# ai-forever/Kandinsky-2

Measured on NVIDIA H100. Metric: unet_denoising_steps_per_sec, higher is better.
Workload: dtype f16

## Files before the change

kandinsky-2_b200/csrc/k2_api.cu:

```cuda
#include <stdio.h>
#include <stdlib.h>
#include <string.h>

#include <algorithm>
#include <atomic>
#include <mutex>

#include "../../include/k2b200.h"
#include "k2_internal.h"

namespace k2 {

static thread_local std::string g_err;
static std::atomic<long long> g_launches{0};
static int g_force_bn = 0;
static int g_force_split = 0;
static int g_pdl = 0;


void set_error(const std::string& msg) { g_err = msg; }
int fail(const std::string& msg) {
  g_err = msg;
  return -1;
}
// ... 77 lines not shown
      for (int k = (tn == 1 ? 0 : 1); k < 2; ++k) {
        bool better = best_tiles[k] < 0 || tiles < best_tiles[k];
        if (!better && tiles == best_tiles[k]) {
          if (tn != bn[k]) {
            better = tn < bn[k];
          } else {
            const int d_new = tw > th ? tw - th : th - tw;
            const int d_old = bw[k] > bh[k] ? bw[k] - bh[k] : bh[k] - bw[k];
            better = (d_new < d_old) || (d_new == d_old && tw > bw[k]);
          }
        }
        if (better) {
          best_tiles[k] = tiles;
          bn[k] = tn;
          bw[k] = tw;
          bh[k] = th;
        }
      }
    }
  }
  const int k = (!single_image_only && best_tiles[1] * 100 <= best_tiles[0] * 85) ? 1 : 0;
  TN = bn[k];
  TW = bw[k];
  TH = bh[k];
}


struct ConvPlan {
  int TN, TH, TW, tiles_w, tiles_h, tiles_n, m_tiles;
  int m_tiles_phase;
  int BN, splits;
  int fuse_stats, row_groups;
  int es;
};

static void plan_conv(int NB, int H, int W, bool any9, int kchunks, int Cout, int out_mode, bool has_workspace,
                      long long workspace_bytes, bool want_gn, ConvPlan& pl, const int* cfg = nullptr, bool up2 = false,
                      bool w_batched = false) {
  const int g_force_bn = (cfg && cfg[0]) ? cfg[0] : k2::g_force_bn;
  const int g_force_split = (cfg && cfg[2]) ? cfg[2] : k2::g_force_split;
  pl.es = (cfg && cfg[3]) ? cfg[3] : k2::g_conv_epi_sets;
  choose_tile(NB, H, W, pl.TN, pl.TH, pl.TW, w_batched);
  pl.tiles_w = (W + pl.TW - 1) / pl.TW;
  pl.tiles_h = (H + pl.TH - 1) / pl.TH;
  pl.tiles_n = (NB + pl.TN - 1) / pl.TN;
  pl.m_tiles = pl.tiles_w * pl.tiles_h * pl.tiles_n;
  pl.m_tiles_phase = pl.m_tiles;

  int BN = g_force_bn;
  int splits = 1;
  const long long M_total = static_cast<long long>(NB) * H * W;
  const bool can_split = !up2 && !w_batched && has_workspace && out_mode == 0 && Cout % 8 == 0;
  auto split_ok = [&](int sp) {
    if (sp == 1) return true;
    const int kps = (kchunks + sp - 1) / sp;
    return can_split && kps >= 8 && (sp - 1) * kps < kchunks &&
           static_cast<long long>(sp) * M_total * Cout * 4 <= workspace_bytes;
  };
  auto model = [&](int bn, int sp) {
    const long long nt = (Cout + bn - 1) / bn;
    const long long units = static_cast<long long>(pl.m_tiles) * nt * sp * (up2 ? 4 : 1);
    const long long slots = num_sms();
    const long long waves = (units + slots - 1) / slots;
    const long long kps = (kchunks + sp - 1) / sp;
    long long cost = waves * (kps * (4LL * bn + 60) + 2000);
    if (sp > 1) cost += 4000 + (static_cast<long long>(sp) + 1) * M_total * Cout * 4 / 1800;
    return cost;
  };
  if (BN == 0) {
    if (Cout <= 16) BN = 16;
    else if (Cout <= 64) BN = 64;
    else if (Cout <= 128) BN = 128;
    else BN = 0;
  }
  {
    const int cand[3] = {256, 192, 128};
    long long best = -1;
    int best_bn = BN ? BN : 256, best_sp = 1;
    for (int ci = 0; ci < 3; ++ci) {
      const int bn = BN ? BN : cand[ci];
      if (BN && ci > 0) break;
      for (int sp = 1; sp <= 8; ++sp) {
        if (g_force_split > 0 && sp != g_force_split) continue;
        if (!split_ok(sp)) continue;
        const long long c = model(bn, sp);
        if (best < 0 || c < best) {
          best = c;
          best_bn = bn;
          best_sp = sp;
        }
      }
    }
    BN = best_bn;
    splits = best_sp;
  }
  pl.BN = BN;
  pl.splits = splits;

  pl.fuse_stats = 0;
  pl.row_groups = 0;
  if (want_gn && out_mode == 0 && Cout % 8 == 0) {
    if (splits == 1 && BN >= 64 && Cout % 64 == 0 && (pl.TN == 1 || pl.TH * pl.TW == 16)) {
      pl.fuse_stats = 1;
      pl.row_groups = ((pl.TN == 1) ? pl.m_tiles : NB * pl.tiles_h * pl.tiles_w) * (up2 ? 4 : 1);
    } else if (splits > 1 && (static_cast<long long>(H) * W) % 16 == 0) {
      pl.fuse_stats = 2;
      pl.row_groups = static_cast<int>(M_total / 16);
    }
  }
}

static void plan_to_info(const ConvPlan& pl, int* info) {
  if (!info) return;
  info[0] = pl.BN; info[1] = 0;
  info[2] = pl.splits; info[3] = pl.m_tiles; info[4] = pl.TN;
  info[5] = pl.fuse_stats; info[6] = pl.row_groups;
}

}

using namespace k2;

extern "C" {

const char* k2_last_error(void) { return g_err.c_str(); }
int k2_version(void) { return 100; }
long long k2_launch_count(void) { return g_launches.load(); }
void k2_reset_launch_count(void) { g_launches.store(0); }
int k2_set_tuning(int key, int value) {
  if (key == 0) {
    g_force_bn = value;
    return 0;
  }
  if (key == 1) {
    g_force_split = value;
    return 0;
  }
  if (key == 2) {
    if (value == 2) return fail("k2_set_tuning: no CTA-pair conv kernel on sm_90");
    return 0;
  }
  if (key == 4) {
    g_pdl = value;
    return 0;
  }
  if (key == 10) {
    g_conv_epi_sets = (value == 2) ? 2 : 1;
    return 0;
  }
  if (key == 11) {
    g_gn_bps = value;
    return 0;
  }
  if (key == 9) {
    return 0;
  }

  return fail("k2_set_tuning: unknown key");
}

int k2_conv_gemm(const K2ConvSrc* srcs, int nsrc, int NB, int H, int W, const void* w_packed, int w_rows,
                 int Ktot, int ldw, int Cout, const float* bias, const void* residual, int ldr, void* out, int ldo,
                 int out_mode, void* workspace, long long workspace_bytes, float* gn_partial, int* info,
                 k2_stream_t stream) {
  return k2_conv_gemm_cfg(srcs, nsrc, NB, H, W, w_packed, w_rows, Ktot, ldw, Cout, bias, residual, ldr, out, ldo, out_mode,
                          workspace, workspace_bytes, gn_partial, info, nullptr, 0, stream);
}

int k2_conv_gemm_cfg(const K2ConvSrc* srcs, int nsrc, int NB, int H, int W, const void* w_packed, int w_rows,
                     int Ktot, int ldw, int Cout, const float* bias, const void* residual, int ldr, void* out, int ldo,
                     int out_mode, void* workspace, long long workspace_bytes, float* gn_partial, int* info,
                     const int* cfg, long long w_batch_stride, k2_stream_t stream) {
  K2_REQUIRE(w_batch_stride >= 0 && w_batch_stride % 8 == 0, "conv_gemm_cfg: w_batch_stride must be a multiple of 8 elements");
  const bool w_batched = w_batch_stride > 0;
  if (cfg) {
    K2_REQUIRE(cfg[0] == 0 || cfg[0] == 16 || cfg[0] == 64 || cfg[0] == 128 || cfg[0] == 192 || cfg[0] == 256,
               "conv_gemm_cfg: N tile must be 0, 16, 64, 128, 192 or 256");
    K2_REQUIRE(cfg[1] >= 0 && cfg[1] <= 2 && cfg[2] >= 0 && cfg[2] <= 8 && cfg[3] >= 0 && cfg[3] <= 2,
               "conv_gemm_cfg: pair mode in 0..2, splits in 0..8, epilogue sets in 0..2");
    K2_REQUIRE(cfg[1] != 2, "conv_gemm_cfg: no CTA-pair conv kernel on sm_90");
  }
  K2_REQUIRE(nsrc >= 1 && nsrc <= 3, "conv_gemm: 1..3 sources");
  K2_REQUIRE((reinterpret_cast<uintptr_t>(gn_partial) & 7) == 0, "conv_gemm: gn_partial must be 8-byte aligned");
  K2_REQUIRE(NB > 0 && H > 0 && W > 0 && Cout > 0, "conv_gemm: bad geometry");
  K2_REQUIRE(w_rows >= Cout, "conv_gemm: w_rows < Cout");
  K2_REQUIRE(Ktot % 64 == 0, "conv_gemm: Ktot must be a multiple of 64");
  if (ldw == 0) ldw = Ktot;
  K2_REQUIRE(ldw >= Ktot && ldw % 8 == 0 && (reinterpret_cast<uintptr_t>(w_packed) & 15) == 0,
             "conv_gemm: weight row stride / alignment");
  ConvGemmParams p;
  memset(&p, 0, sizeof p);
  p.NB = NB;
  p.H = H;
  p.W = W;
  bool any9 = false;
  int kchunks = 0;
  const bool up2 = srcs[0].taps == 4;
  if (up2) {
    K2_REQUIRE(nsrc == 1 && out_mode == 0 && residual == nullptr && H % 2 == 0 && W % 2 == 0,
               "conv_gemm: a taps == 4 source (3x3 conv over its nearest-2x upsampling) must be the only source, with fp16 "
               "output, no residual and even output H, W");
    H /= 2;
    W /= 2;
    p.H = H;
    p.W = W;
  }
  for (int s = 0; s < nsrc; ++s) {
    const K2ConvSrc& src = srcs[s];
    K2_REQUIRE(src.taps == 9 || src.taps == 1 || (s == 0 && src.taps == 4), "conv_gemm: taps must be 9 or 1 (or 4: up2)");
    K2_REQUIRE(src.C > 0 && src.C % 8 == 0 && src.ld % 8 == 0 && src.ld >= src.C, "conv_gemm: bad source C/ld");
    K2_REQUIRE((reinterpret_cast<uintptr_t>(src.ptr) & 15) == 0, "conv_gemm: source not 16B aligned");
    any9 = any9 || src.taps == 9;
    p.seg_taps[s] = src.taps;
// ... 26 lines not shown
                        static_cast<uint64_t>(NB)};
    uint64_t str[3] = {static_cast<uint64_t>(src.ld) * 2, static_cast<uint64_t>(src.ld) * 2 * W,
                       static_cast<uint64_t>(src.ld) * 2 * W * H};
    uint32_t box[4] = {64, static_cast<uint32_t>(p.TW), static_cast<uint32_t>(p.TH), static_cast<uint32_t>(p.TN)};
    if (encode_tmap_f16(&p.tmA[s], src.ptr, 4, dims, str, box)) return -1;
  }
  const int BN = pl.BN, splits = pl.splits, fuse_stats = pl.fuse_stats;
  p.splits = splits;
  p.k_per_split = (kchunks + splits - 1) / splits;
  p.M_total = static_cast<long long>(NB) * H * W * (up2 ? 4 : 1);
  p.ws = reinterpret_cast<float*>(workspace);
  p.n_tiles = (Cout + BN - 1) / BN;
  p.Cout = Cout;
  {
    uint64_t dims[3] = {static_cast<uint64_t>(Ktot), static_cast<uint64_t>(w_rows), static_cast<uint64_t>(w_batched ? NB : 1)};
    uint64_t str[2] = {static_cast<uint64_t>(ldw) * 2,
                       (w_batched ? static_cast<uint64_t>(w_batch_stride) : static_cast<uint64_t>(ldw) * w_rows) * 2};
    uint32_t box[3] = {64, static_cast<uint32_t>(BN), 1};
    if (encode_tmap_f16(&p.tmB, w_packed, 3, dims, str, box)) return -1;
  }
  p.bias = bias;
  p.residual = reinterpret_cast<const __half*>(residual);
  p.ldr = ldr;
  p.out = out;
  p.ldo = ldo;
  p.out_mode = (splits > 1) ? 2 : out_mode;
  p.gn_part = (fuse_stats == 1) ? reinterpret_cast<float2*>(gn_partial) : nullptr;
  p.gn_mode = (fuse_stats == 1) ? (p.TN == 1 ? 1 : 2) : 0;
  if (out_mode == 0) {
    K2_REQUIRE(ldo % 8 == 0 && (reinterpret_cast<uintptr_t>(out) & 15) == 0, "conv_gemm: out alignment");
    if (residual)
      K2_REQUIRE(ldr % 8 == 0 && (reinterpret_cast<uintptr_t>(residual) & 15) == 0, "conv_gemm: residual alignment");
  }
  int rc = launch_conv_gemm(p, BN, pl.es, static_cast<cudaStream_t>(stream));
  if (rc == 0) g_launches.fetch_add(1, std::memory_order_relaxed);
  if (rc == 0 && splits > 1) {
    rc = launch_splitk_finalize(p.ws, splits, p.M_total, Cout, bias, p.residual, ldr, reinterpret_cast<__half*>(out), ldo,
                                fuse_stats == 2 ? reinterpret_cast<float2*>(gn_partial) : nullptr,
                                static_cast<cudaStream_t>(stream));
    if (rc == 0) g_launches.fetch_add(1, std::memory_order_relaxed);
  }
  return rc;
}

int k2_conv_plan(int NB, int H, int W, int taps, int Ktot, int Cout, int out_mode, long long workspace_bytes,
                 int want_gn_partial, int* info) {
  K2_REQUIRE(NB > 0 && H > 0 && W > 0 && Cout > 0 && info, "conv_plan: bad arguments");
  K2_REQUIRE(Ktot > 0 && Ktot % 64 == 0, "conv_plan: Ktot must be a positive multiple of 64");
  ConvPlan pl;
  plan_conv(NB, H, W, taps == 9, Ktot / 64, Cout, out_mode, workspace_bytes > 0, workspace_bytes, want_gn_partial != 0, pl);
  plan_to_info(pl, info);
  return 0;
}

}
```

kandinsky-2_b200/csrc/k2_conv_gemm.cu:

```cuda
#include <stdio.h>

#include "k2_common.cuh"
#include "k2_internal.h"

namespace k2 {

namespace {

constexpr int BM = 128;
constexpr int BK = 64;
constexpr int A_STAGE_BYTES = BM * BK * 2;
constexpr int ACC_PAD = 4;

constexpr int EPI_STAGE_FLOATS = 32 * 33;
constexpr int EPI_BYTES = 4 * EPI_STAGE_FLOATS * 4 + 4 * 256 * 4;
constexpr int SMEM_LIMIT = 227 * 1024;

template <int BN, int ES>
struct Cfg {
  static constexpr int B_STAGE_BYTES = BN * BK * 2;
  static constexpr int STAGE_BYTES = A_STAGE_BYTES + B_STAGE_BYTES;
  static constexpr int BNC = (BN < 64) ? BN : (ES == 2 ? 128 : 64);
  static_assert(ES == 1 || BN % 128 == 0, "two epilogue sets need N tiles of 128 or 256");
  static constexpr int ACC_BYTES = BM * (BNC + ACC_PAD) * 4;
// ... 280 lines not shown
                uint4 ov;
                __half2* oh = reinterpret_cast<__half2*>(&ov);
#pragma unroll
                for (int e = 0; e < 4; ++e) oh[e] = __floats2half2_rn(f[2 * e], f[2 * e + 1]);
                *reinterpret_cast<uint4*>(orow + v * 8) = ov;
              }
            } else {
#pragma unroll
              for (int e = 0; e < CH; ++e) {
                if (col0 + e < p.Cout) {
                  float f = __uint_as_float(r[e]);
                  if (p.bias) f += __ldg(p.bias + col0 + e);
                  if (rrow) f += __half2float(rrow[e]);
                  orow[e] = __float2half_rn(f);
                }
              }
            }
          } else {
            float* o = reinterpret_cast<float*>(p.out);
#pragma unroll
            for (int e = 0; e < CH; ++e) {
              if (col0 + e < p.Cout) {
                float f = __uint_as_float(r[e]);
                if (p.bias) f += __ldg(p.bias + col0 + e);
                o[((static_cast<long long>(n) * p.Cout + (col0 + e)) * p.H + y) * p.W + x] = f;
              }
            }
          }
        }
      }
}


template <int BN, int ES>
__global__ void __launch_bounds__(384, 1) conv_gemm_kernel(const __grid_constant__ ConvGemmParams p) {
  using C = Cfg<BN, ES>;
  constexpr int BNC = C::BNC;
  constexpr int NA = BN / 2;
  extern __shared__ uint8_t smem_raw[];
  uint8_t* smem = reinterpret_cast<uint8_t*>((reinterpret_cast<uintptr_t>(smem_raw) + 1023) &
                                             ~static_cast<uintptr_t>(1023));
  float* acc_smem = reinterpret_cast<float*>(smem + C::STAGES * C::STAGE_BYTES);
  float* stat_smem = reinterpret_cast<float*>(smem + C::STAGES * C::STAGE_BYTES + C::ACC_BYTES);
  uint64_t* full_bar = reinterpret_cast<uint64_t*>(smem + C::STAGES * C::STAGE_BYTES + C::ACC_BYTES + ES * EPI_BYTES);
  uint64_t* empty_bar = full_bar + C::STAGES;

  const int warp_idx = threadIdx.x >> 5;
  const int lane = threadIdx.x & 31;
  const int wg = warp_idx >> 2;

  if (threadIdx.x == 0) {
    tma_prefetch_desc(&p.tmB);
    for (int s = 0; s < 3; ++s)
      if (p.seg_taps[s]) tma_prefetch_desc(&p.tmA[s]);
    for (int i = 0; i < C::STAGES; ++i) {
      mbar_init(&full_bar[i], 1);
      mbar_init(&empty_bar[i], 8);
    }
    fence_barrier_init();
  }
  __syncthreads();
  pdl_wait();
  pdl_launch();

  const int total_tiles = p.m_tiles * p.n_tiles * p.splits;

  if (wg == 0) {
    setmaxnreg_dec<40>();
    if (warp_idx == 0 && elect_one()) {
      int stage = 0;
      uint32_t ring_phase = 0;
      const uint32_t tx_bytes = p.a_box_bytes + C::B_STAGE_BYTES;
      for (int tile = blockIdx.x; tile < total_tiles; tile += gridDim.x) {
        const int m_idx = tile % p.m_tiles;
        const int n_idx = (tile / p.m_tiles) % p.n_tiles;
        const int split = tile / (p.m_tiles * p.n_tiles);
        int n0, y0, x0, phase;
        decode_m_tile(p, m_idx, n0, y0, x0, phase);
        const int kb = phase * p.num_k_chunks;
        const int k0 = split * p.k_per_split;
        const int k1 = min(p.num_k_chunks, k0 + p.k_per_split);
        int s = 0, rem = k0;
        while (rem >= p.seg_taps[s] * p.seg_kchunks[s]) {
          rem -= p.seg_taps[s] * p.seg_kchunks[s];
          ++s;
        }
        int tap = rem / p.seg_kchunks[s];
        int c = rem - tap * p.seg_kchunks[s];
        for (int kc = k0; kc < k1; ++kc) {
          const int taps = p.seg_taps[s];
          const int dy = (taps == 9) ? (tap / 3 - 1) : (taps == 4 ? (tap >> 1) + (phase >> 1) - 1 : 0);
          const int dx = (taps == 9) ? (tap % 3 - 1) : (taps == 4 ? (tap & 1) + (phase & 1) - 1 : 0);
          mbar_wait_lean(&empty_bar[stage], ring_phase ^ 1);
          uint8_t* sA = smem + stage * C::STAGE_BYTES;
          uint8_t* sB = sA + A_STAGE_BYTES;
          mbar_arrive_expect_tx(&full_bar[stage], tx_bytes);
          tma_load_4d(sA, &p.tmA[s], &full_bar[stage], c * BK, x0 + dx, y0 + dy, n0);
          tma_load_3d(sB, &p.tmB, &full_bar[stage], (kb + kc) * BK, n_idx * BN, p.w_batched ? n0 : 0);
          if (++stage == C::STAGES) {
            stage = 0;
            ring_phase ^= 1;
          }
          if (++c == p.seg_kchunks[s]) {
            c = 0;
            if (++tap == taps) {
              tap = 0;
              ++s;
            }
          }
        }
      }
    }
  } else {
    setmaxnreg_inc<232>();
    const int g = wg - 1;
    const int w = warp_idx & 3;
    int stage = 0;
    uint32_t phase = 0;
    for (int tile = blockIdx.x; tile < total_tiles; tile += gridDim.x) {
      const int m_idx = tile % p.m_tiles;
      const int n_idx = (tile / p.m_tiles) % p.n_tiles;
      const int split = tile / (p.m_tiles * p.n_tiles);
      const int nk = min(p.num_k_chunks, (split + 1) * p.k_per_split) - split * p.k_per_split;
      float acc[NA];
#pragma unroll
      for (int i = 0; i < NA; ++i) acc[i] = 0.f;
      int prev_stage = -1;
      for (int kc = 0; kc < nk; ++kc) {
        mbar_wait_lean(&full_bar[stage], phase);
        const uint32_t a_addr = smem_u32(smem + stage * C::STAGE_BYTES) + g * (64 * 128);
        const uint32_t b_addr = smem_u32(smem + stage * C::STAGE_BYTES + A_STAGE_BYTES);
        wgmma_fence();
#pragma unroll
        for (int k = 0; k < BK / 16; ++k) {
          const uint64_t adesc = make_wgmma_desc(a_addr) + static_cast<uint64_t>(k * 2);
          const uint64_t bdesc = make_wgmma_desc(b_addr) + static_cast<uint64_t>(k * 2);
          if constexpr (BN == 256) {
            wgmma_m64n256k16(acc, adesc, bdesc, 1u);
          } else if constexpr (BN == 192) {
            wgmma_m64n192k16(acc, adesc, bdesc, 1u);
          } else if constexpr (BN == 128) {
            wgmma_m64n128k16(acc, adesc, bdesc, 1u);
          } else if constexpr (BN == 64) {
            wgmma_m64n64k16(acc, adesc, bdesc, 1u);
          } else {
            static_assert(BN == 16, "conv_gemm: N tile without a wgmma shape");
            wgmma_m64n16k16(acc, adesc, bdesc, 1u);
          }
        }
        wgmma_commit();
        wgmma_wait<1>();
        if (prev_stage >= 0 && lane == 0) mbar_arrive(&empty_bar[prev_stage]);
        prev_stage = stage;
        if (++stage == C::STAGES) {
          stage = 0;
          phase ^= 1;
        }
      }
      wgmma_wait<0>();
      if (prev_stage >= 0 && lane == 0) mbar_arrive(&empty_bar[prev_stage]);

      int n0, y0, x0, mphase;
      decode_m_tile(p, m_idx, n0, y0, x0, mphase);
      const int r0 = 64 * g + 16 * w + (lane >> 2);
      const int cq = 2 * (lane & 3);
#pragma unroll
      for (int pass = 0; pass < BN / BNC; ++pass) {
        named_bar_sync(3, 256);
#pragma unroll
        for (int i = 0; i < NA; i += 2) {
          if ((8 * (i >> 2)) / BNC != pass) continue;
          const int row = r0 + 8 * ((i >> 1) & 1);
          const int col = 8 * (i >> 2) - pass * BNC + cq;
          *reinterpret_cast<float2*>(acc_smem + row * (BNC + ACC_PAD) + col) = make_float2(acc[i], acc[i + 1]);
        }
        named_bar_sync(3, 256);
        if (ES == 2 || g == 0)
          epilogue_tile<BNC, ES>(p, acc_smem, w, lane, n0, y0, x0, n_idx * BN + pass * BNC, split, m_idx, stat_smem, g,
                                 mphase);
      }
    }
  }
}

__global__ void __launch_bounds__(256) splitk_finalize_kernel(const float* __restrict__ ws, int splits, long long M,
                                                              int Cout, const float* __restrict__ bias,
                                                              const __half* __restrict__ residual, int ldr,
                                                              __half* __restrict__ out, int ldo, float2* __restrict__ gn_part) {
  __shared__ float red[8][32][17];
  const int vx = threadIdx.x & 31, ry = threadIdx.x >> 5;
  const int c0 = (blockIdx.y * 32 + vx) * 8;
  const long long rg = blockIdx.x;
  pdl_wait();
  pdl_launch();
  float st[16];
#pragma unroll
  for (int e = 0; e < 16; ++e) st[e] = 0.f;
  if (c0 < Cout) {
    float bv[8];
#pragma unroll
    for (int e = 0; e < 8; ++e) bv[e] = bias ? __ldg(bias + c0 + e) : 0.f;
#pragma unroll
    for (int rr = 0; rr < 2; ++rr) {
      const long long m = rg * 16 + ry + rr * 8;
      if (m >= M) continue;
      float f[8];
#pragma unroll
      for (int e = 0; e < 8; ++e) f[e] = bv[e];
      for (int s = 0; s < splits; ++s) {
        const float4* w = reinterpret_cast<const float4*>(ws + (static_cast<long long>(s) * M + m) * Cout + c0);
        const float4 a = __ldcs(w), b = __ldcs(w + 1);
        f[0] += a.x; f[1] += a.y; f[2] += a.z; f[3] += a.w; f[4] += b.x; f[5] += b.y; f[6] += b.z; f[7] += b.w;
      }
// ... 9 lines not shown
      }
      uint4 ov;
      __half2* oh = reinterpret_cast<__half2*>(&ov);
#pragma unroll
      for (int e = 0; e < 4; ++e) {
        oh[e] = __floats2half2_rn(f[2 * e], f[2 * e + 1]);
        const float2 t = __half22float2(oh[e]);
        st[2 * e] += t.x;
        st[2 * e + 1] += t.y;
        st[8 + 2 * e] = fmaf(t.x, t.x, st[8 + 2 * e]);
        st[8 + 2 * e + 1] = fmaf(t.y, t.y, st[8 + 2 * e + 1]);
      }
      *reinterpret_cast<uint4*>(out + m * ldo + c0) = ov;
    }
  }
  if (gn_part == nullptr) return;
#pragma unroll
  for (int e = 0; e < 16; ++e) red[ry][vx][e] = st[e];
  __syncthreads();
  const int vx2 = threadIdx.x >> 3, e2 = threadIdx.x & 7;
  const int c = (blockIdx.y * 32 + vx2) * 8 + e2;
  if (c < Cout) {
    float s1 = 0.f, s2 = 0.f;
#pragma unroll
    for (int q = 0; q < 8; ++q) {
      s1 += red[q][vx2][e2];
      s2 += red[q][vx2][8 + e2];
    }
    gn_part[rg * Cout + c] = make_float2(s1, s2);
  }
}


template <int BN, int ES>
int launch_bn(const ConvGemmParams& p, cudaStream_t stream) {
  using C = Cfg<BN, ES>;
  static bool attr_set = false;
  if (!attr_set) {
    K2_CHECK_CUDA(cudaFuncSetAttribute(conv_gemm_kernel<BN, ES>, cudaFuncAttributeMaxDynamicSharedMemorySize,
                                       C::SMEM_BYTES));
    attr_set = true;
  }
  int total = p.m_tiles * p.n_tiles * p.splits;
  int grid = total < num_sms() ? total : num_sms();
  K2_CHECK_CUDA(launch_k(conv_gemm_kernel<BN, ES>, dim3(grid), dim3(384), C::SMEM_BYTES, stream, p));
  return 0;
}

}

int launch_splitk_finalize(const float* ws, int splits, long long M, int Cout, const float* bias, const __half* residual,
                           int ldr, __half* out, int ldo, float2* gn_part, cudaStream_t stream) {
  dim3 grid(static_cast<unsigned int>((M + 15) / 16), (Cout / 8 + 31) / 32);
  K2_CHECK_CUDA(launch_k(splitk_finalize_kernel, grid, dim3(256), 0, stream, ws, splits, M, Cout, bias, residual, ldr, out, ldo,
                         gn_part));
  return 0;
}

int launch_conv_gemm(const ConvGemmParams& p, int BN, int epilogue_sets, cudaStream_t stream) {
  if (epilogue_sets == 2) {
    switch (BN) {
      case 128: return launch_bn<128, 2>(p, stream);
      case 256: return launch_bn<256, 2>(p, stream);
      default: break;
    }
  }
  switch (BN) {
    case 16: return launch_bn<16, 1>(p, stream);
    case 64: return launch_bn<64, 1>(p, stream);
    case 128: return launch_bn<128, 1>(p, stream);
    case 192: return launch_bn<192, 1>(p, stream);
    case 256: return launch_bn<256, 1>(p, stream);
    default: return fail("conv_gemm: unsupported BN");
  }
}

}
```

kandinsky-2_b200/csrc/k2_internal.h:

```cpp
#pragma once
#include <cuda.h>
#include <cuda_fp16.h>
#include <cuda_runtime.h>
#include <stdint.h>

#include <string>

namespace k2 {

void set_error(const std::string& msg);
int fail(const std::string& msg);
#define K2_CHECK_CUDA(expr)                                                                 \
  do {                                                                                      \
    cudaError_t _e = (expr);                                                                \
    if (_e != cudaSuccess)                                                                  \
      return ::k2::fail(std::string(#expr) + ": " + cudaGetErrorString(_e));                \
  } while (0)
#define K2_REQUIRE(cond, msg)                                  \
  do {                                                         \
    if (!(cond)) return ::k2::fail(std::string("k2b200: ") + (msg)); \
  } while (0)

inline bool aligned16(const void* p) { return (reinterpret_cast<uintptr_t>(p) & 15) == 0; }

// ... 18 lines not shown
void count_launch(int n = 1);

int encode_tmap_f16(CUtensorMap* out, const void* base, int rank, const uint64_t* dims,
                    const uint64_t* strides_bytes , const uint32_t* box);

struct ConvGemmParams {
  CUtensorMap tmA[3];
  CUtensorMap tmB;
  int w_batched;
  int seg_taps[3];
  int seg_kchunks[3];
  int num_k_chunks;
  int NB, H, W;
  int TN, TH, TW;
  int tiles_n, tiles_h, tiles_w;
  int m_tiles, n_tiles;
  int Cout;
  const float* bias;
  const __half* residual;
  int ldr;
  void* out;
  int ldo;
  int out_mode;
  uint32_t a_box_bytes;
  int splits;
  int k_per_split;
  float* ws;
  long long M_total;
  float2* gn_part;
  int gn_mode;
  int up2;
  int m_tiles_phase;
};
int launch_conv_gemm(const ConvGemmParams& p, int BN, int epilogue_sets, cudaStream_t stream);
int launch_splitk_finalize(const float* ws, int splits, long long M, int Cout, const float* bias, const __half* residual,
                           int ldr, __half* out, int ldo, float2* gn_part, cudaStream_t stream);

struct FlashParams {
  const __half* qkv;
  long long ldq;
  int hs, q_off, k_off, v_off;
  const __half* enc;
  long long lde;
  int ehs, ek_off, ev_off;
  int B, heads, T, Tc;
  __half* out;
  int ldo, ohs;
  float scale_log2e;
};
int gn_apply_blocks_per_sm();
int launch_attention(const FlashParams& p, int head_dim, cudaStream_t stream);

}
```

kandinsky-2_b200/kandinsky2/launch_plan.py:

```python
import os

import torch

from . import ops

FOLD_MAX_RG = int(os.environ.get("K2_GN_FOLD_MAX_RG", "18"))
TUNE = os.environ.get("K2_AUTOTUNE", "1") != "0"
FORK = os.environ.get("K2_FORK", "1") != "0"
TUNE_SMALL_M = int(os.environ.get("K2_TUNE_SMALL_M", "8192"))
_tune_cache = {}


def tune(key, run, m_rows=0):
    if not TUNE:
        return None
    key = (torch.cuda.current_device(), TUNE_SMALL_M) + key
    if key in _tune_cache:
        return _tune_cache[key]
    info = [0] * 7
    run(None, info)
    bn0, splits = info[0], info[2]
    cout = key[3]
    best = None
    if cout > 64:
        bns = [bn0] if splits > 1 else [bn for bn in (128, 192, 256) if bn - 64 < cout or bn == bn0]
        cands = [(bn0, 0, splits, 1)] + [(bn, 0, splits, es) for bn in bns for es in ((1,) if bn == 192 else (1, 2))
                                        if (bn, es) != (bn0, 1)]
        if 0 < m_rows <= TUNE_SMALL_M and splits == 1:
            for bn in (128, 192, 256):
                if bn - 64 >= cout:
                    continue
                for sp in (2, 3, 4):
                    probe = [0] * 7
                    try:
                        run((bn, 1, sp, 1), probe)
                    except Exception:
                        continue
                    if probe[0] == bn and probe[2] == sp:
                        cands.append((bn, 1, sp, 1))

        def timed(cfg, reps=6):
            run(cfg)
            evs = [torch.cuda.Event(enable_timing=True) for _ in range(reps + 1)]
            evs[0].record()
            for i in range(reps):
                run(cfg)
                evs[i + 1].record()
            torch.cuda.synchronize()
            return min(evs[i].elapsed_time(evs[i + 1]) for i in range(reps))

        t0 = tb = timed(cands[0])
        for cfg in cands[1:]:
            t = timed(cfg)
            if t < tb and t < 0.97 * t0:
                t = max(t, timed(cfg))
                if t < tb and t < 0.97 * t0:
                    best, tb = cfg, t
    _tune_cache[key] = best
    return best


class LaunchPlan:
    def __init__(self, dev, nb):
        self.dev = dev
        self.NB = nb
        self._parts = {}
        self._scratch = {}
        self.steps = []
        self.graph = None
        self._side_stream = None
        self._side_open = False
        self._serial = False
# ... 149 lines not shown
```

kandinsky-2_b200/kandinsky2/ops.py:

```python
import ctypes

import torch

from . import _native as nat
from ._native import K2ConvSrc, check, ptr, stream_ptr


def _row_stride(t):
    assert t.stride(-1) == 1, "channel dim must be contiguous"
    ld = t.stride(-2)
    n = t.shape[-2]
    for d in range(t.dim() - 3, -1, -1):
        assert t.shape[d] == 1 or t.stride(d) == ld * n, f"not a row-strided NHWC view: {t.shape} {t.stride()}"
        n *= t.shape[d]
    return ld


def _pad64(c):
    return (c + 63) // 64 * 64


def pack_conv_weight(w, split=None):
    w = w.detach()
    if w.dim() == 2:
# ... 46 lines not shown


def _workspace(dev):
    buf = _conv_ws.get(dev.index)
    if buf is None:
        buf = torch.empty(_CONV_WS_BYTES, dtype=torch.uint8, device=dev)
        _conv_ws[dev.index] = buf
    return buf


def conv_gemm(srcs, w_packed, cout, bias=None, residual=None, out=None, out_mode=0, geom=None, gn_part=None, info=None,
              cfg=None, w_batch_stride=0):
    lib = nat.load()
    t0 = srcs[0][0]
    NB, H, W = geom if geom is not None else t0.shape[:3]
    if srcs[0][1] == 4:
        H, W = 2 * H, 2 * W
    arr = (K2ConvSrc * len(srcs))()
    for i, (t, taps) in enumerate(srcs):
        assert t.dtype == torch.float16 and t.is_cuda
        arr[i].ptr = t.data_ptr()
        arr[i].C = t.shape[-1]
        arr[i].ld = _row_stride(t)
        arr[i].taps = taps
    if out is None:
        if out_mode == 0:
            out = torch.empty((NB, H, W, cout), dtype=torch.float16, device=t0.device)
        else:
            out = torch.empty((NB, cout, H, W), dtype=torch.float32, device=t0.device)
    ldo = _row_stride(out) if out_mode == 0 else 0
    ldr = _row_stride(residual) if residual is not None else 0
    assert w_packed.dtype == torch.float16 and w_packed.stride(1) == 1
    ws = _workspace(t0.device)
    _info = (ctypes.c_int * 7)()
    _cfg = (ctypes.c_int * 4)(*cfg) if cfg is not None else None
    check(lib.k2_conv_gemm_cfg(arr, len(srcs), NB, H, W, ptr(w_packed), w_packed.shape[0], w_packed.shape[1],
                               w_packed.stride(0), cout,
                               ptr(bias), ptr(residual), ldr, ptr(out), ldo, out_mode, ptr(ws), ws.numel(), ptr(gn_part),
                               _info, _cfg, int(w_batch_stride), stream_ptr()))
    if info is not None:
        info[:] = list(_info)
    return out


def conv_plan(NB, H, W, taps, ktot, cout, out_mode=0, workspace_bytes=_CONV_WS_BYTES, want_gn_partial=True):
    lib = nat.load()
    info = (ctypes.c_int * 7)()
    check(lib.k2_conv_plan(NB, H, W, taps, ktot, cout, out_mode, workspace_bytes, int(want_gn_partial), info))
    keys = ("n_tile", "cta_pair", "splits", "m_tiles", "images_per_tile", "gn_partial_mode", "row_groups")
    return dict(zip(keys, list(info)))


def gemm_rows(x, w_packed, cout, bias=None, residual=None, out=None, cfg=None, info=None):
    lead = x.shape[:-1]
    M = 1
    for d in lead:
        M *= d
    x3 = x.reshape(1, 1, M, x.shape[-1]) if x.is_contiguous() else None
    if x3 is None:
        x3 = x.as_strided((1, 1, M, x.shape[-1]), (0, 0, x.stride(-2), 1))
    if out is None:
        out = torch.empty(tuple(lead) + (cout,), dtype=torch.float16, device=x.device)
    o3 = out.as_strided((1, 1, M, cout), (0, 0, out.stride(-2), 1))
    r3 = None
    if residual is not None:
        r3 = residual.as_strided((1, 1, M, cout), (0, 0, residual.stride(-2), 1))
    conv_gemm([(x3, 1)], w_packed, cout, bias=bias, residual=r3, out=o3, geom=(1, 1, M), cfg=cfg, info=info)
    return out


_gn_scratch = {}


_GN_SCRATCH_FLOATS = 1 << 23


def _scratch(dev, nfloats):
    key = (dev.index, )
    buf = _gn_scratch.get(key)
    if buf is None:
# ... 397 lines not shown
```

profiles/conv_layers.py:

```python
import argparse
import json
import os
import subprocess
import sys

ROOT = os.path.dirname(os.path.dirname(os.path.abspath(__file__)))
for p in (ROOT, os.path.join(ROOT, "kandinsky-2_b200")):
    if p not in sys.path:
        sys.path.insert(0, p)

import torch

B, H, W = 4, 96, 96


def _card():
    q = subprocess.run(["nvidia-smi", "--query-gpu=name,power.limit,clocks.max.sm", "--format=csv,noheader", "-i", "0"],
                       capture_output=True, text=True)
    return q.stdout.strip() or torch.cuda.get_device_name(0)


def _pad64(c):
    return (c + 63) // 64 * 64

# ... 8 lines not shown
        M, K = x.numel() // xshape[-1], xshape[-1]
        w = rnd(cout, K)
        bias = torch.randn(cout, device=dev, generator=g)
        res = rnd(*xshape[:-1], cout) if has_res else None
        out = torch.empty(*xshape[:-1], cout, device=dev, dtype=torch.float16)
        run = lambda cfg, info=None: ops.gemm_rows(x, w, cout, bias=bias, residual=res, out=out, cfg=cfg, info=info)
        return run, dict(M=M, N=cout, K=K, desc=f"gemm {M}x{K}->{cout}" + (" +res" if has_res else ""))
    _, _, oshape, geom, srcs_spec, has_res, has_part, out_mode, w_batched = key
    if w_batched:
        return None, None
    if geom is not None:
        NB, Ho, Wo = geom
    elif out_mode == 0:
        NB, Ho, Wo = oshape[:3]
    else:
        NB, Ho, Wo = oshape[0], oshape[2], oshape[3]
    up2 = srcs_spec[0][1] == 4
    Hs, Ws = (Ho // 2, Wo // 2) if up2 else (Ho, Wo)
    srcs = [(rnd(NB, Hs, Ws, c), taps) for c, taps in srcs_spec]
    K = sum(taps * _pad64(c) for c, taps in srcs_spec)
    w_rows = max(16, cout)
    w = rnd(w_rows, 4 * K if up2 else K)
    bias = torch.randn(cout, device=dev, generator=g)
    res = rnd(NB, Ho, Wo, cout) if has_res else None
    out = torch.empty(*oshape, device=dev, dtype=torch.float16 if out_mode == 0 else torch.float32)
    part = torch.zeros(ops.gn_part_floats(NB, Ho, Wo, cout), device=dev) if has_part else None
    run = lambda cfg, info=None: ops.conv_gemm(srcs, w, cout, bias=bias, residual=res, out=out, out_mode=out_mode, geom=geom,
                                               gn_part=part, cfg=cfg, info=info)
    desc = (f"{NB}x{Ho}x{Wo} " + "+".join(f"{c}{'x3x3' if t == 9 else ('up2' if t == 4 else 'x1x1')}" for c, t in srcs_spec)
            + f"->{cout}" + (" +res" if has_res else "") + (" fp32-nchw" if out_mode else ""))
    return run, dict(M=NB * Ho * Wo, N=cout, K=K, desc=desc)


def _time(run, cfg, min_ms):
    for _ in range(3):
        run(cfg)
    torch.cuda.synchronize()
    s, e = torch.cuda.Event(enable_timing=True), torch.cuda.Event(enable_timing=True)
    s.record()
    for _ in range(5):
        run(cfg)
    e.record()
    torch.cuda.synchronize()
    reps = max(10, int(min_ms / max(s.elapsed_time(e) / 5, 1e-3)) + 1)
    s.record()
    for _ in range(reps):
        run(cfg)
    e.record()
    torch.cuda.synchronize()
    return s.elapsed_time(e) / reps, reps


def main():
    ap = argparse.ArgumentParser()
    ap.add_argument("--out", default=None)
    ap.add_argument("--min-ms", type=float, default=50.0, help="timed window per configuration")
    ap.add_argument("--mma-n", default="tile", choices=["tile", "64"],
                    help="wgmma N of the build: one instruction per N tile, or m64n64k16 per 64 columns")
    args = ap.parse_args()
    if not torch.cuda.is_available():
        raise SystemExit("needs a CUDA sm_90 device")
    import bench
    from kandinsky2 import launch_plan, ops
    from kandinsky2.model.gaussian_diffusion import FusedStep, create_ddpm_v22
    dev = torch.device("cuda", 0)
    torch.cuda.set_device(dev)
    ops.set_tuning(4, 1)
    res = {"card": _card(), "torch": torch.__version__, "geometry": f"cfg-2: UNet batch {2 * B}, {H}x{W} latents",
           "mma_n": args.mma_n, "min_ms": args.min_ms}

    counts = {}
    tune = launch_plan.tune

    def counting_tune(key, run, m_rows=0):
        counts[key] = counts.get(key, 0) + 1
        return tune(key, run, m_rows=m_rows)
    launch_plan.tune = counting_tune
    model = bench.build_unet(dev)
    image_emb = torch.randn(2 * B, 1280, generator=torch.Generator().manual_seed(1234)).to(dev)
    step = FusedStep(model, B, H, W, dict(image_emb=image_emb), guidance_scale=4.0, cond_first=False, clip_range=2.0,
                     threshold_mode=0)
    launch_plan.tune = tune
    diffusion = create_ddpm_v22(50)
    coef, ts = diffusion._tables(dev)
    order = torch.arange(diffusion.num_timesteps - 1, -1, -1, device=dev)
    step.set_schedule(ts[order], coef[order], torch.randn(len(order), B, 4, H, W, device=dev))
    x = step.latent()
    x.copy_(torch.randn(B, 4, H, W, device=dev))
    step.advance(x)
    torch.cuda.synchronize()
    res["plan_conv_launches"] = sum(1 for _, kind, _ in step.plan.steps if kind == "conv_gemm")
    res["counted_conv_launches"] = sum(counts.values())

    g = torch.Generator(device=dev).manual_seed(7)
    layers = []
    for key, n in counts.items():
        run, shp = _layer(key, dev, g)
        if run is None:
            continue
        info = [0] * 7
        picked = launch_plan._tune_cache.get((dev.index, launch_plan.TUNE_SMALL_M) + key)
        run(picked, info)
        picked_cfg = [info[0], 0, info[2], (picked[3] if picked and picked[3] else 1)]
        cout = shp["N"]
        cfgs = []
        if cout > 64:
            cfgs = [(bn, 0, 1, es) for bn in (128, 192, 256) if bn - 64 < cout or bn == info[0]
                    for es in ((1,) if bn == 192 else (1, 2))]
        if tuple(picked_cfg) not in cfgs:
            cfgs.append(tuple(picked_cfg))
        rows = []
        for cfg in cfgs:
            info = [0] * 7
            run(cfg, info)
            bn, splits = info[0], info[2]
            ms, reps = _time(run, cfg, args.min_ms)
            flops = 2.0 * shp["M"] * cout * shp["K"]
            mma_n = bn if (args.mma_n == "tile" or bn < 64) else 64
            smem_bpf = (2048 + 32 * mma_n) / (2.0 * 64 * mma_n * 16)
            m_tiles = info[3] * (4 if "up2" in shp["desc"] else 1)
            chunks = m_tiles * ((cout + bn - 1) // bn) * (shp["K"] // 64)
            l2_bytes = chunks * (16384 + bn * 128)
            rows.append(dict(n_tile=bn, epilogue_sets=cfg[3], splits=splits, ms=round(ms, 5), reps=reps,
                             tflops=round(flops / (ms * 1e-3) / 1e12, 1),
                             smem_operand_bytes_per_flop=round(smem_bpf, 5),
                             l2_operand_bytes_per_flop=round(l2_bytes / flops, 5),
                             l2_operand_TBps=round(l2_bytes / (ms * 1e-3) / 1e12, 2)))
        pick = next((r for r in rows if [r["n_tile"], r["splits"], r["epilogue_sets"]] ==
                     [picked_cfg[0], picked_cfg[2], picked_cfg[3]]), rows[0])
        layers.append(dict(shape=shp["desc"], key=repr(key), launches_per_step=n, gemm_gflop=round(2e-9 * shp["M"] * cout * shp["K"], 3),
                           picked=dict(n_tile=picked_cfg[0], splits=picked_cfg[2], epilogue_sets=picked_cfg[3],
                                       tuned=picked is not None),
                           picked_ms=pick["ms"], configs=rows))
    total = sum(l["launches_per_step"] * l["picked_ms"] for l in layers)
    for l in layers:
        l["share_of_conv_time"] = round(l["launches_per_step"] * l["picked_ms"] / total, 4)
    layers.sort(key=lambda l: -l["share_of_conv_time"])
    res["conv_ms_per_step_at_picked"] = round(total, 3)
    res["layers"] = layers

    print(f"# {res['card']}  (mma_n={args.mma_n})  conv time per step at the picked configurations: {total:.2f} ms")
    print(f"{'shape':44s} {'n':>2s} {'share':>6s} {'pick':>9s}  " + "  ".join(f"{c:>9s}" for c in
          ("128/1", "128/2", "192/1", "256/1", "256/2")) + "   (TFLOP/s at N tile / epilogue sets, splits 1)")
    for l in layers:
        by = {(r["n_tile"], r["epilogue_sets"]): r["tflops"] for r in l["configs"] if r["splits"] == 1}
        pk = l["picked"]
        print(f"{l['shape'][:44]:44s} {l['launches_per_step']:2d} {100 * l['share_of_conv_time']:5.1f}% "
              f"{pk['n_tile']:>3d}/{pk['epilogue_sets']}/{pk['splits']:<3d}  " +
              "  ".join(f"{by.get(c, float('nan')):9.1f}" for c in ((128, 1), (128, 2), (192, 1), (256, 1), (256, 2))))
    if args.out:
        os.makedirs(os.path.dirname(os.path.abspath(args.out)), exist_ok=True)
        with open(args.out, "w") as f:
            f.write(json.dumps(res, indent=1) + "\n")


if __name__ == "__main__":
    main()
```

Before: 29.71.

## Add ping-pong warpgroup schedule for N-tile-128 conv GEMM

Adds a ping-pong variant of the persistent conv GEMM kernel. Two consumer warpgroups alternate whole tiles, each computing a 128-row tile with two m64 accumulators, and take turns on the MMA and epilogue phases through named barriers, so one group's epilogue overlaps the other's tensor-core work. The variant becomes the default whenever the planner picks N tile 128 with one epilogue set, and the Python autotuner and profiling script gain it as a candidate. It doubles accumulator registers per thread and adds inter-warpgroup barrier handoffs.

```diff
diff --git a/kandinsky-2_b200/csrc/k2_api.cu b/kandinsky-2_b200/csrc/k2_api.cu
--- a/kandinsky-2_b200/csrc/k2_api.cu
+++ b/kandinsky-2_b200/csrc/k2_api.cu
@@ -133,6 +133,7 @@
   int BN, splits;
   int fuse_stats, row_groups;
   int es;
+  int sched;
 };
 
 static void plan_conv(int NB, int H, int W, bool any9, int kchunks, int Cout, int out_mode, bool has_workspace,
@@ -197,6 +198,9 @@
   }
   pl.BN = BN;
   pl.splits = splits;
+  if (cfg && cfg[4]) pl.sched = cfg[4];
+  else pl.sched = (BN == 128 && pl.es == 1 && !(cfg && cfg[3])) ? 2 : 1;
+  if (pl.sched == 2) pl.es = 1;
 
   pl.fuse_stats = 0;
   pl.row_groups = 0;
@@ -216,6 +220,7 @@
   info[0] = pl.BN; info[1] = 0;
   info[2] = pl.splits; info[3] = pl.m_tiles; info[4] = pl.TN;
   info[5] = pl.fuse_stats; info[6] = pl.row_groups;
+  info[7] = pl.sched;
 }
 
 }
@@ -280,6 +285,9 @@
     K2_REQUIRE(cfg[1] >= 0 && cfg[1] <= 2 && cfg[2] >= 0 && cfg[2] <= 8 && cfg[3] >= 0 && cfg[3] <= 2,
                "conv_gemm_cfg: pair mode in 0..2, splits in 0..8, epilogue sets in 0..2");
     K2_REQUIRE(cfg[1] != 2, "conv_gemm_cfg: no CTA-pair conv kernel on sm_90");
+    K2_REQUIRE(cfg[4] >= 0 && cfg[4] <= 2, "conv_gemm_cfg: schedule in 0..2");
+    K2_REQUIRE(cfg[4] != 2 || (cfg[0] == 128 && cfg[3] != 2),
+               "conv_gemm_cfg: the ping-pong schedule runs N tile 128 with one epilogue set per warpgroup");
   }
   K2_REQUIRE(nsrc >= 1 && nsrc <= 3, "conv_gemm: 1..3 sources");
   K2_REQUIRE((reinterpret_cast<uintptr_t>(gn_partial) & 7) == 0, "conv_gemm: gn_partial must be 8-byte aligned");
@@ -372,7 +380,7 @@
     if (residual)
       K2_REQUIRE(ldr % 8 == 0 && (reinterpret_cast<uintptr_t>(residual) & 15) == 0, "conv_gemm: residual alignment");
   }
-  int rc = launch_conv_gemm(p, BN, pl.es, static_cast<cudaStream_t>(stream));
+  int rc = launch_conv_gemm(p, BN, pl.es, pl.sched, static_cast<cudaStream_t>(stream));
   if (rc == 0) g_launches.fetch_add(1, std::memory_order_relaxed);
   if (rc == 0 && splits > 1) {
     rc = launch_splitk_finalize(p.ws, splits, p.M_total, Cout, bias, p.residual, ldr, reinterpret_cast<__half*>(out), ldo,
diff --git a/kandinsky-2_b200/csrc/k2_conv_gemm.cu b/kandinsky-2_b200/csrc/k2_conv_gemm.cu
--- a/kandinsky-2_b200/csrc/k2_conv_gemm.cu
+++ b/kandinsky-2_b200/csrc/k2_conv_gemm.cu
@@ -336,11 +336,36 @@
 }
 
 
-template <int BN, int ES>
+__device__ __forceinline__ void sts_v2(uint32_t saddr, float a, float b) {
+  asm volatile("st.shared.v2.f32 [%0], {%1, %2};" ::"r"(saddr), "f"(a), "f"(b) : "memory");
+}
+
+template <int BN>
+__device__ __forceinline__ void wgmma_tile(float (&acc)[BN / 2], uint64_t adesc, uint64_t bdesc) {
+  if constexpr (BN == 256) {
+    wgmma_m64n256k16(acc, adesc, bdesc, 1u);
+  } else if constexpr (BN == 192) {
+    wgmma_m64n192k16(acc, adesc, bdesc, 1u);
+  } else if constexpr (BN == 128) {
+    wgmma_m64n128k16(acc, adesc, bdesc, 1u);
+  } else if constexpr (BN == 64) {
+    wgmma_m64n64k16(acc, adesc, bdesc, 1u);
+  } else {
+    static_assert(BN == 16, "conv_gemm: N tile without a wgmma shape");
+    wgmma_m64n16k16(acc, adesc, bdesc, 1u);
+  }
+}
+
+constexpr int PP_STAGE_BAR = 2;
+constexpr int PP_MMA_TURN = 4;
+constexpr int PP_EPI_TURN = 6;
+
+template <int BN, int ES, bool PP>
 __global__ void __launch_bounds__(384, 1) conv_gemm_kernel(const __grid_constant__ ConvGemmParams p) {
   using C = Cfg<BN, ES>;
   constexpr int BNC = C::BNC;
   constexpr int NA = BN / 2;
+  static_assert(!PP || ES == 1, "ping-pong: each warpgroup drains its own tiles");
   extern __shared__ uint8_t smem_raw[];
   uint8_t* smem = reinterpret_cast<uint8_t*>((reinterpret_cast<uintptr_t>(smem_raw) + 1023) &
                                              ~static_cast<uintptr_t>(1023));
@@ -359,7 +384,7 @@
       if (p.seg_taps[s]) tma_prefetch_desc(&p.tmA[s]);
     for (int i = 0; i < C::STAGES; ++i) {
       mbar_init(&full_bar[i], 1);
-      mbar_init(&empty_bar[i], 8);
+      mbar_init(&empty_bar[i], PP ? 4 : 8);
     }
     fence_barrier_init();
   }
@@ -415,7 +440,7 @@
         }
       }
     }
-  } else {
+  } else if constexpr (!PP) {
     setmaxnreg_inc<232>();
     const int g = wg - 1;
     const int w = warp_idx & 3;
@@ -439,18 +464,7 @@
         for (int k = 0; k < BK / 16; ++k) {
           const uint64_t adesc = make_wgmma_desc(a_addr) + static_cast<uint64_t>(k * 2);
           const uint64_t bdesc = make_wgmma_desc(b_addr) + static_cast<uint64_t>(k * 2);
-          if constexpr (BN == 256) {
-            wgmma_m64n256k16(acc, adesc, bdesc, 1u);
-          } else if constexpr (BN == 192) {
-            wgmma_m64n192k16(acc, adesc, bdesc, 1u);
-          } else if constexpr (BN == 128) {
-            wgmma_m64n128k16(acc, adesc, bdesc, 1u);
-          } else if constexpr (BN == 64) {
-            wgmma_m64n64k16(acc, adesc, bdesc, 1u);
-          } else {
-            static_assert(BN == 16, "conv_gemm: N tile without a wgmma shape");
-            wgmma_m64n16k16(acc, adesc, bdesc, 1u);
-          }
+          wgmma_tile<BN>(acc, adesc, bdesc);
         }
         wgmma_commit();
         wgmma_wait<1>();
@@ -483,6 +497,80 @@
           epilogue_tile<BNC, ES>(p, acc_smem, w, lane, n0, y0, x0, n_idx * BN + pass * BNC, split, m_idx, stat_smem, g,
                                  mphase);
       }
+    }
+  } else {
+    setmaxnreg_inc<232>();
+    const int g = wg - 1;
+    const int w = warp_idx & 3;
+    const int ntiles = (total_tiles - static_cast<int>(blockIdx.x) + static_cast<int>(gridDim.x) - 1) / static_cast<int>(gridDim.x);
+    if (g == 1) {
+      named_bar_arrive(PP_MMA_TURN, 256);
+      named_bar_arrive(PP_EPI_TURN, 256);
+    }
+    int stage = 0;
+    uint32_t phase = 0;
+    for (int j = 0; j < ntiles; ++j) {
+      const int tile = blockIdx.x + j * gridDim.x;
+      const int m_idx = tile % p.m_tiles;
+      const int n_idx = (tile / p.m_tiles) % p.n_tiles;
+      const int split = tile / (p.m_tiles * p.n_tiles);
+      const int nk = min(p.num_k_chunks, (split + 1) * p.k_per_split) - split * p.k_per_split;
+      if ((j & 1) != g) {
+        const int s2 = stage + max(nk, 0);
+        phase ^= static_cast<uint32_t>((s2 / C::STAGES) & 1);
+        stage = s2 % C::STAGES;
+        continue;
+      }
+      float acc0[NA], acc1[NA];
+#pragma unroll
+      for (int i = 0; i < NA; ++i) {
+        acc0[i] = 0.f;
+        acc1[i] = 0.f;
+      }
+      named_bar_sync(PP_MMA_TURN + g, 256);
+      int prev_stage = -1;
+      for (int kc = 0; kc < nk; ++kc) {
+        mbar_wait_lean(&full_bar[stage], phase);
+        const uint32_t a_addr = smem_u32(smem + stage * C::STAGE_BYTES);
+        const uint32_t b_addr = smem_u32(smem + stage * C::STAGE_BYTES + A_STAGE_BYTES);
+        wgmma_fence();
+#pragma unroll
+        for (int k = 0; k < BK / 16; ++k) {
+          const uint64_t bdesc = make_wgmma_desc(b_addr) + static_cast<uint64_t>(k * 2);
+          wgmma_tile<BN>(acc0, make_wgmma_desc(a_addr) + static_cast<uint64_t>(k * 2), bdesc);
+          wgmma_tile<BN>(acc1, make_wgmma_desc(a_addr + 64 * 128) + static_cast<uint64_t>(k * 2), bdesc);
+        }
+        wgmma_commit();
+        wgmma_wait<1>();
+        if (prev_stage >= 0 && lane == 0) mbar_arrive(&empty_bar[prev_stage]);
+        prev_stage = stage;
+        if (++stage == C::STAGES) {
+          stage = 0;
+          phase ^= 1;
+        }
+      }
+      if (j + 1 < ntiles) named_bar_arrive(PP_MMA_TURN + 1 - g, 256);
+      wgmma_wait<0>();
+      if (prev_stage >= 0 && lane == 0) mbar_arrive(&empty_bar[prev_stage]);
+
+      int n0, y0, x0, mphase;
+      decode_m_tile(p, m_idx, n0, y0, x0, mphase);
+      const uint32_t st0 = smem_u32(acc_smem + (16 * w + (lane >> 2)) * (BNC + ACC_PAD) + 2 * (lane & 3));
+      named_bar_sync(PP_EPI_TURN + g, 256);
+#pragma unroll
+      for (int pass = 0; pass < BN / BNC; ++pass) {
+        if (pass > 0) named_bar_sync(PP_STAGE_BAR + g, 128);
+#pragma unroll
+        for (int i = 0; i < NA; i += 2) {
+          if ((8 * (i >> 2)) / BNC != pass) continue;
+          const uint32_t off = (8 * ((i >> 1) & 1) * (BNC + ACC_PAD) + 8 * (i >> 2) - pass * BNC) * 4;
+          sts_v2(st0 + off, acc0[i], acc0[i + 1]);
+          sts_v2(st0 + off + 64 * (BNC + ACC_PAD) * 4, acc1[i], acc1[i + 1]);
+        }
+        named_bar_sync(PP_STAGE_BAR + g, 128);
+        epilogue_tile<BNC, 1>(p, acc_smem, w, lane, n0, y0, x0, n_idx * BN + pass * BNC, split, m_idx, stat_smem, 0, mphase);
+      }
+      if (j + 1 < ntiles) named_bar_arrive(PP_EPI_TURN + 1 - g, 256);
     }
   }
 }
@@ -558,18 +646,18 @@
 }
 
 
-template <int BN, int ES>
+template <int BN, int ES, bool PP = false>
 int launch_bn(const ConvGemmParams& p, cudaStream_t stream) {
   using C = Cfg<BN, ES>;
   static bool attr_set = false;
   if (!attr_set) {
-    K2_CHECK_CUDA(cudaFuncSetAttribute(conv_gemm_kernel<BN, ES>, cudaFuncAttributeMaxDynamicSharedMemorySize,
+    K2_CHECK_CUDA(cudaFuncSetAttribute(conv_gemm_kernel<BN, ES, PP>, cudaFuncAttributeMaxDynamicSharedMemorySize,
                                        C::SMEM_BYTES));
     attr_set = true;
   }
   int total = p.m_tiles * p.n_tiles * p.splits;
   int grid = total < num_sms() ? total : num_sms();
-  K2_CHECK_CUDA(launch_k(conv_gemm_kernel<BN, ES>, dim3(grid), dim3(384), C::SMEM_BYTES, stream, p));
+  K2_CHECK_CUDA(launch_k(conv_gemm_kernel<BN, ES, PP>, dim3(grid), dim3(384), C::SMEM_BYTES, stream, p));
   return 0;
 }
 
@@ -583,7 +671,11 @@
   return 0;
 }
 
-int launch_conv_gemm(const ConvGemmParams& p, int BN, int epilogue_sets, cudaStream_t stream) {
+int launch_conv_gemm(const ConvGemmParams& p, int BN, int epilogue_sets, int schedule, cudaStream_t stream) {
+  if (schedule == 2) {
+    if (BN == 128 && epilogue_sets == 1) return launch_bn<128, 1, true>(p, stream);
+    return fail("conv_gemm: the ping-pong schedule runs N tile 128 with one epilogue set per warpgroup");
+  }
   if (epilogue_sets == 2) {
     switch (BN) {
       case 128: return launch_bn<128, 2>(p, stream);
diff --git a/kandinsky-2_b200/csrc/k2_internal.h b/kandinsky-2_b200/csrc/k2_internal.h
--- a/kandinsky-2_b200/csrc/k2_internal.h
+++ b/kandinsky-2_b200/csrc/k2_internal.h
@@ -74,7 +74,7 @@
   int up2;
   int m_tiles_phase;
 };
-int launch_conv_gemm(const ConvGemmParams& p, int BN, int epilogue_sets, cudaStream_t stream);
+int launch_conv_gemm(const ConvGemmParams& p, int BN, int epilogue_sets, int schedule, cudaStream_t stream);
 int launch_splitk_finalize(const float* ws, int splits, long long M, int Cout, const float* bias, const __half* residual,
                            int ldr, __half* out, int ldo, float2* gn_part, cudaStream_t stream);
 
diff --git a/kandinsky-2_b200/kandinsky2/launch_plan.py b/kandinsky-2_b200/kandinsky2/launch_plan.py
--- a/kandinsky-2_b200/kandinsky2/launch_plan.py
+++ b/kandinsky-2_b200/kandinsky2/launch_plan.py
@@ -17,27 +17,28 @@
     key = (torch.cuda.current_device(), TUNE_SMALL_M) + key
     if key in _tune_cache:
         return _tune_cache[key]
-    info = [0] * 7
+    info = [0] * 8
     run(None, info)
-    bn0, splits = info[0], info[2]
+    bn0, splits, sched0 = info[0], info[2], info[7]
     cout = key[3]
     best = None
     if cout > 64:
         bns = [bn0] if splits > 1 else [bn for bn in (128, 192, 256) if bn - 64 < cout or bn == bn0]
-        cands = [(bn0, 0, splits, 1)] + [(bn, 0, splits, es) for bn in bns for es in ((1,) if bn == 192 else (1, 2))
-                                        if (bn, es) != (bn0, 1)]
+        variants = [(bn, es, 1) for bn in bns for es in ((1,) if bn == 192 else (1, 2))] + [(128, 1, 2) for bn in bns if bn == 128]
+        cands = [(bn0, 0, splits, 1, sched0)] + [(bn, 0, splits, es, sc) for bn, es, sc in variants
+                                                 if (bn, es, sc) != (bn0, 1, sched0)]
         if 0 < m_rows <= TUNE_SMALL_M and splits == 1:
-            for bn in (128, 192, 256):
+            for bn, sc in ((128, 1), (128, 2), (192, 1), (256, 1)):
                 if bn - 64 >= cout:
                     continue
                 for sp in (2, 3, 4):
-                    probe = [0] * 7
+                    probe = [0] * 8
                     try:
-                        run((bn, 1, sp, 1), probe)
+                        run((bn, 1, sp, 1, sc), probe)
                     except Exception:
                         continue
                     if probe[0] == bn and probe[2] == sp:
-                        cands.append((bn, 1, sp, 1))
+                        cands.append((bn, 1, sp, 1, sc))
 
         def timed(cfg, reps=6):
             run(cfg)
diff --git a/kandinsky-2_b200/kandinsky2/ops.py b/kandinsky-2_b200/kandinsky2/ops.py
--- a/kandinsky-2_b200/kandinsky2/ops.py
+++ b/kandinsky-2_b200/kandinsky2/ops.py
@@ -102,8 +102,8 @@
     ldr = _row_stride(residual) if residual is not None else 0
     assert w_packed.dtype == torch.float16 and w_packed.stride(1) == 1
     ws = _workspace(t0.device)
-    _info = (ctypes.c_int * 7)()
-    _cfg = (ctypes.c_int * 4)(*cfg) if cfg is not None else None
+    _info = (ctypes.c_int * 8)()
+    _cfg = (ctypes.c_int * 5)(*cfg) if cfg is not None else None
     check(lib.k2_conv_gemm_cfg(arr, len(srcs), NB, H, W, ptr(w_packed), w_packed.shape[0], w_packed.shape[1],
                                w_packed.stride(0), cout,
                                ptr(bias), ptr(residual), ldr, ptr(out), ldo, out_mode, ptr(ws), ws.numel(), ptr(gn_part),
@@ -115,7 +115,7 @@
 
 def conv_plan(NB, H, W, taps, ktot, cout, out_mode=0, workspace_bytes=_CONV_WS_BYTES, want_gn_partial=True):
     lib = nat.load()
-    info = (ctypes.c_int * 7)()
+    info = (ctypes.c_int * 8)()
     check(lib.k2_conv_plan(NB, H, W, taps, ktot, cout, out_mode, workspace_bytes, int(want_gn_partial), info))
     keys = ("n_tile", "cta_pair", "splits", "m_tiles", "images_per_tile", "gn_partial_mode", "row_groups")
     return dict(zip(keys, list(info)))
diff --git a/profiles/conv_layers.py b/profiles/conv_layers.py
--- a/profiles/conv_layers.py
+++ b/profiles/conv_layers.py
@@ -64,6 +64,34 @@
     return run, dict(M=NB * Ho * Wo, N=cout, K=K, desc=desc)
 
 
+def _sched(info):
+    return info[7] if len(info) > 7 else 1
+
+
+def _fits(layers, sms):
+    fam = {}
+    for l in layers:
+        for r in l["configs"]:
+            if r["splits"] != 1:
+                continue
+            name = f"{r['n_tile']}/{'pp' if r['schedule'] == 2 else r['epilogue_sets']}"
+            fam.setdefault((name, l["M"], l["N"], r["tiles"]), {})[r["k_chunks"]] = r["ms"] * 1e3
+    out = []
+    for (name, M, N, tiles), pts in sorted(fam.items()):
+        if len(pts) < 2:
+            continue
+        ks = sorted(pts)
+        n = len(ks)
+        mk = sum(ks) / n
+        mt = sum(pts[k] for k in ks) / n
+        a = sum((k - mk) * (pts[k] - mt) for k in ks) / sum((k - mk) ** 2 for k in ks)
+        b = mt - a * mk
+        rounds = (tiles + sms - 1) // sms
+        out.append(dict(config=name, M=M, N=N, tiles=tiles, rounds=rounds, k_chunks=ks,
+                        us_per_chunk_per_round=round(a / rounds, 4), fixed_us_per_round=round(b / rounds, 2)))
+    return out
+
+
 def _time(run, cfg, min_ms):
     for _ in range(3):
         run(cfg)
@@ -130,21 +158,26 @@
         run, shp = _layer(key, dev, g)
         if run is None:
             continue
-        info = [0] * 7
+        info = [0] * 8
         picked = launch_plan._tune_cache.get((dev.index, launch_plan.TUNE_SMALL_M) + key)
         run(picked, info)
-        picked_cfg = [info[0], 0, info[2], (picked[3] if picked and picked[3] else 1)]
+        picked_cfg = [info[0], 0, info[2], (picked[3] if picked and picked[3] else 1), _sched(info)]
         cout = shp["N"]
         cfgs = []
         if cout > 64:
-            cfgs = [(bn, 0, 1, es) for bn in (128, 192, 256) if bn - 64 < cout or bn == info[0]
-                    for es in ((1,) if bn == 192 else (1, 2))]
+            cfgs = [(bn, 0, 1, es, 1) for bn in (128, 192, 256) if bn - 64 < cout or bn == info[0]
+                    for es in ((1,) if bn == 192 else (1, 2))] + [(128, 0, 1, 1, 2)]
         if tuple(picked_cfg) not in cfgs:
             cfgs.append(tuple(picked_cfg))
         rows = []
         for cfg in cfgs:
-            info = [0] * 7
-            run(cfg, info)
+            info = [0] * 8
+            if cfg[4] == 1:
+                cfg = cfg[:4]
+            try:
+                run(cfg, info)
+            except (IndexError, RuntimeError):
+                continue
             bn, splits = info[0], info[2]
             ms, reps = _time(run, cfg, args.min_ms)
             flops = 2.0 * shp["M"] * cout * shp["K"]
@@ -153,16 +186,18 @@
             m_tiles = info[3] * (4 if "up2" in shp["desc"] else 1)
             chunks = m_tiles * ((cout + bn - 1) // bn) * (shp["K"] // 64)
             l2_bytes = chunks * (16384 + bn * 128)
-            rows.append(dict(n_tile=bn, epilogue_sets=cfg[3], splits=splits, ms=round(ms, 5), reps=reps,
+            rows.append(dict(n_tile=bn, epilogue_sets=cfg[3], schedule=_sched(info), splits=splits, ms=round(ms, 5), reps=reps,
+                             tiles=m_tiles * ((cout + bn - 1) // bn), k_chunks=shp["K"] // 64,
                              tflops=round(flops / (ms * 1e-3) / 1e12, 1),
                              smem_operand_bytes_per_flop=round(smem_bpf, 5),
                              l2_operand_bytes_per_flop=round(l2_bytes / flops, 5),
                              l2_operand_TBps=round(l2_bytes / (ms * 1e-3) / 1e12, 2)))
-        pick = next((r for r in rows if [r["n_tile"], r["splits"], r["epilogue_sets"]] ==
-                     [picked_cfg[0], picked_cfg[2], picked_cfg[3]]), rows[0])
+        pick = next((r for r in rows if [r["n_tile"], r["splits"], r["epilogue_sets"], r["schedule"]] ==
+                     [picked_cfg[0], picked_cfg[2], picked_cfg[3], picked_cfg[4]]), rows[0])
         layers.append(dict(shape=shp["desc"], key=repr(key), launches_per_step=n, gemm_gflop=round(2e-9 * shp["M"] * cout * shp["K"], 3),
+                           M=shp["M"], N=cout,
                            picked=dict(n_tile=picked_cfg[0], splits=picked_cfg[2], epilogue_sets=picked_cfg[3],
-                                       tuned=picked is not None),
+                                       schedule=picked_cfg[4], tuned=picked is not None),
                            picked_ms=pick["ms"], configs=rows))
     total = sum(l["launches_per_step"] * l["picked_ms"] for l in layers)
     for l in layers:
@@ -170,16 +205,23 @@
     layers.sort(key=lambda l: -l["share_of_conv_time"])
     res["conv_ms_per_step_at_picked"] = round(total, 3)
     res["layers"] = layers
+    res["fixed_cost_fits"] = _fits(layers, torch.cuda.get_device_properties(dev).multi_processor_count)
 
     print(f"# {res['card']}  (mma_n={args.mma_n})  conv time per step at the picked configurations: {total:.2f} ms")
-    print(f"{'shape':44s} {'n':>2s} {'share':>6s} {'pick':>9s}  " + "  ".join(f"{c:>9s}" for c in
-          ("128/1", "128/2", "192/1", "256/1", "256/2")) + "   (TFLOP/s at N tile / epilogue sets, splits 1)")
+    cols = ((128, 1, 1), (128, 2, 1), (128, 1, 2), (192, 1, 1), (256, 1, 1), (256, 2, 1))
+    print(f"{'shape':44s} {'n':>2s} {'share':>6s} {'pick':>11s}  " + "  ".join(f"{c:>9s}" for c in
+          ("128/1", "128/2", "128/pp", "192/1", "256/1", "256/2")) + "   (TFLOP/s at N tile / epilogue sets, splits 1)")
     for l in layers:
-        by = {(r["n_tile"], r["epilogue_sets"]): r["tflops"] for r in l["configs"] if r["splits"] == 1}
+        by = {(r["n_tile"], r["epilogue_sets"], r["schedule"]): r["tflops"] for r in l["configs"] if r["splits"] == 1}
         pk = l["picked"]
         print(f"{l['shape'][:44]:44s} {l['launches_per_step']:2d} {100 * l['share_of_conv_time']:5.1f}% "
-              f"{pk['n_tile']:>3d}/{pk['epilogue_sets']}/{pk['splits']:<3d}  " +
-              "  ".join(f"{by.get(c, float('nan')):9.1f}" for c in ((128, 1), (128, 2), (192, 1), (256, 1), (256, 2))))
+              f"{pk['n_tile']:>3d}/{pk['epilogue_sets']}/{pk['splits']}/{'pp' if pk['schedule'] == 2 else 'co'}  " +
+              "  ".join(f"{by.get(c, float('nan')):9.1f}" for c in cols))
+    print("# per-tile-round cost fits (time = a * chunks + b over same M / N / tiles, different K):")
+    for f in res["fixed_cost_fits"]:
+        print(f"  {f['config']:>10s}  M {f['M']:6d} N {f['N']:5d} tiles {f['tiles']:5d} rounds {f['rounds']:3d}  "
+              f"{f['us_per_chunk_per_round']:.3f} us/chunk/round  {f['fixed_us_per_round']:6.2f} us/round  "
+              f"over chunks {f['k_chunks']}")
     if args.out:
         os.makedirs(os.path.dirname(os.path.abspath(args.out)), exist_ok=True)
         with open(args.out, "w") as f:
```

New measurement: 30.04 (median of 6 runs). 1.1% higher.
